# Ghostish/ObjectCentricOccCompletion

Measured on AMD Instinct MI355X. Metric: object-grids/sec (fwd+bwd), higher is better.
Workload: dtype bf16; 1 GPU; configs[1]: SubMConv3d-only occupancy encoder fwd+bwd+AdamW, 64 object grids/GPU x 2000 random points, 0.2 m voxels, 40^3 grid, channels 16-32-64-128, LN+GELU, bf16 features; grids_per_gpu=64, points_per_grid=2000, active_voxels=126005, rulebook_pairs=221211, parallelism=dp1, launch=one hipGraphLaunch per step

## Files before the change

### objectcentricocccompletion_amd/csrc/grid_geometry.hip

```cpp
#include "common.hpp"
#include "row_order.hpp"

namespace {

#ifdef OCOCC_GEO_STAMPS
__device__ long long* g_stamps = nullptr;
#define STAMP(slot) do { if (threadIdx.x == 0 && g_stamps) g_stamps[(int64_t)blockIdx.x * 16 + (slot)] = (long long)__builtin_amdgcn_s_memrealtime(); } while (0)
#else
#define STAMP(slot) do { } while (0)
#endif

constexpr int kThreads = 1024;
constexpr int kWaves = kThreads / 64;
constexpr int kEmitThreads = 256;
constexpr int kEmitWaves = kEmitThreads / 64;
constexpr int kFusedBasesMaxEntries = 256;
#ifndef OCOCC_GEO_FUSED_BASES
#define OCOCC_GEO_FUSED_BASES 1
#endif
constexpr int kPadBlocks = 64;
constexpr int kCols = 28;
constexpr int kMaxSlices = 16;
constexpr int kCodesPerThread = 8;

#define LDS_BARRIER() asm volatile("s_waitcnt lgkmcnt(0)\n\ts_barrier" ::: "memory")

struct GeoParams {
  float vx, vy, vz, xmin, ymin, zmin;
  int32_t gx, gy, gz, batch;
  int32_t words;
  int32_t slices;
  int32_t wps;
  int32_t asplit;
  int32_t spa;
};

__device__ __forceinline__ int32_t lds_rank(const uint32_t* bm, const uint32_t* pf, int32_t cell) {
  const uint32_t w = bm[cell >> 5];
  const uint32_t bit = 1u << (cell & 31);
  return (w & bit) ? (int32_t)(pf[cell >> 5] + __popc(w & (bit - 1u))) : -1;
}

__device__ void lds_popc_scan(const uint32_t* bm, uint32_t* pf, int words, uint32_t* tmp) {
  const int lane = threadIdx.x & 63, wave = threadIdx.x >> 6;
  uint32_t carry = 0;
  for (int w0 = 0; w0 < words; w0 += kThreads) {
    const int w = w0 + threadIdx.x;
    const uint32_t v = w < words ? (uint32_t)__popc(bm[w]) : 0u;
    uint32_t inc = v;
#pragma unroll
    for (int d = 1; d < 64; d <<= 1) {
      const uint32_t t = __shfl_up(inc, d, 64);
      if (lane >= d) inc += t;
    }
    if (lane == 63) tmp[wave] = inc;
    __syncthreads();
    uint32_t before = 0, total = 0;
    for (int t = 0; t < kWaves; ++t) {
      const uint32_t s = tmp[t];
      if (t < wave) before += s;
      total += s;
    }
    if (w < words) pf[w] = carry + before + inc - v;
    carry += total;
    __syncthreads();
  }
}

__device__ void segment_bounds(const int32_t* __restrict__ batch_idx, int64_t n, int32_t key, int64_t* s_two,
                               int64_t* lo_out, int64_t* hi_out) {
  const int64_t step = (n + kThreads - 1) / kThreads;
  if (threadIdx.x < 2) s_two[threadIdx.x] = n;
  __syncthreads();
  {
    const int64_t c0 = (int64_t)threadIdx.x * step;
    if (c0 < n) {
      const int32_t last = batch_idx[(c0 + step < n ? c0 + step : n) - 1];
      const int32_t prev = c0 > 0 ? batch_idx[c0 - 1] : INT32_MIN;
      if (last >= key && prev < key) s_two[0] = c0;
      if (last >= key + 1 && prev < key + 1) s_two[1] = c0;
    }
  }
  __syncthreads();
  const int64_t b0 = s_two[0], b1 = s_two[1];
  __syncthreads();
  if (threadIdx.x < 2) s_two[threadIdx.x] = n;
  __syncthreads();
  for (int64_t t = threadIdx.x; t < 2 * step; t += kThreads) {
    const int which = t >= step;
    const int64_t base = which ? b1 : b0;
    const int64_t i = base + (which ? t - step : t);
    if (base < n && i < n) {
      const int32_t kk = key + which;
      if (batch_idx[i] >= kk && (i == 0 || batch_idx[i - 1] < kk)) s_two[which] = i;
// ... 151 lines not shown
    int32_t v[8], sum = 0;
#pragma unroll
    for (int j = 0; j < 8; ++j) {
      const int64_t e = e0 + (int64_t)lane * 8 + j;
      v[j] = e < entries ? table[e * kCols + c] : 0;
    }
#pragma unroll
    for (int j = 0; j < 8; ++j) sum += v[j];
    int32_t inc = sum;
#pragma unroll
    for (int d = 1; d < 64; d <<= 1) {
      const int32_t t = __shfl_up(inc, d, 64);
      if (lane >= d) inc += t;
    }
    int32_t run = carry + inc - sum;
#pragma unroll
    for (int j = 0; j < 8; ++j) {
      const int64_t e = e0 + (int64_t)lane * 8 + j;
      if (e < entries) bases[e * kCols + c] = run;
      run += v[j];
    }
    carry += __shfl(inc, 63, 64);
  }
  if (lane == 0) {
    totals[c] = carry;
    if (c < 27) indice_num[26 - c] = carry;
    else *num_voxels = (int32_t)(carry < cap ? carry : cap);
  }
}

__device__ __forceinline__ void put_feat_row(const float* __restrict__ src, float* __restrict__ dst_f32,
                                             uint16_t* __restrict__ dst_bf16, int c, float scale) {
  if ((c & 3) == 0) {
    for (int c0 = 0; c0 < c; c0 += 4) {
      float4 v = *(const float4*)(src + c0);
      v.x *= scale; v.y *= scale; v.z *= scale; v.w *= scale;
      *(float4*)(dst_f32 + c0) = v;
      if (dst_bf16) {
        uint2 q;
        q.x = (uint32_t)ococc_f32_to_bf16(v.x) | ((uint32_t)ococc_f32_to_bf16(v.y) << 16);
        q.y = (uint32_t)ococc_f32_to_bf16(v.z) | ((uint32_t)ococc_f32_to_bf16(v.w) << 16);
        *(uint2*)(dst_bf16 + c0) = q;
      }
    }
  } else {
    for (int ch = 0; ch < c; ++ch) {
      const float v = src[ch] * scale;
      dst_f32[ch] = v;
      if (dst_bf16) dst_bf16[ch] = ococc_f32_to_bf16(v);
    }
  }
}

__global__ void __launch_bounds__(kEmitThreads)
grid_emit_kernel(const float* __restrict__ feats, int c, int64_t n, GeoParams g, const uint32_t* __restrict__ bitmap,
                 const uint32_t* __restrict__ local_prefix, uint32_t* __restrict__ prefix_out,
                 int32_t* __restrict__ code_of, const int64_t* __restrict__ seg, const int32_t* __restrict__ bases,
                 const int32_t* __restrict__ totals, int32_t* __restrict__ inv, int32_t* __restrict__ out_coors,
                 int32_t* __restrict__ counts, float* __restrict__ out_f32, uint16_t* __restrict__ out_bf16, int64_t cap,
                 int32_t* __restrict__ nbr_t, uint32_t* __restrict__ blockmask, int32_t* __restrict__ pairs,
                 int emit_blocks, uint32_t* __restrict__ order_hist, i32x4_t* __restrict__ order_rowrec,
                 const int32_t* __restrict__ count_table, const int32_t* __restrict__ part_sums, int32_t* __restrict__ indice_num,
                 int32_t* __restrict__ num_voxels,
                 const int32_t* __restrict__ bad_flags, int nflags, int32_t* __restrict__ status) {
  extern __shared__ uint32_t smem[];
  __shared__ int32_t s_part[3][kEmitWaves][32];
  __shared__ uint32_t s_oh[kLocalBuckets];
  if ((int)blockIdx.x >= emit_blocks) {
    int64_t total;
    if (part_sums) {
      int32_t v = 0;
      for (int e = threadIdx.x; e < g.batch * g.asplit; e += kEmitThreads) v += part_sums[(int64_t)e * kCols + 27];
#pragma unroll
      for (int d = 32; d >= 1; d >>= 1) v += __shfl_xor(v, d, 64);
      if ((threadIdx.x & 63) == 0) s_part[0][threadIdx.x >> 6][0] = v;
      __syncthreads();
      total = 0;
      for (int w = 0; w < kEmitWaves; ++w) total += s_part[0][w][0];
    } else {
      total = totals[27];
    }
    const int64_t turn = (int64_t)(gridDim.x - emit_blocks) * kEmitThreads;
    const int64_t r0 = total + (int64_t)(blockIdx.x - emit_blocks) * kEmitThreads;
    if (r0 >= cap) return;
    for (int64_t r = r0 + threadIdx.x; r - threadIdx.x < cap; r += turn) {
      const bool have = r < cap;
      if (have) {
        *(int4*)(out_coors + r * 4) = make_int4(-1, -1, -1, -1);
        counts[r] = 0;
        for (int ch = 0; ch < c; ++ch) {
          out_f32[r * c + ch] = 0.f;
          if (out_bf16) out_bf16[r * c + ch] = 0;
        }
        for (int k = 0; k < 27; ++k) nbr_t[(int64_t)k * cap + r] = -1;
      }
      if (order_hist) {
        const int key = order_global(order_key_local(0u, 13), (int)blockIdx.x);
        const unsigned long long m = __ballot(have);
        if (m) {
          const int leader = __ffsll((long long)m) - 1;
          uint32_t first = 0u;
          if ((int)(threadIdx.x & 63) == leader) first = atomicAdd(&order_hist[key], (uint32_t)__popcll(m));
          first = __shfl(first, leader, 64);
          const uint32_t place = first + (uint32_t)__builtin_amdgcn_mbcnt_hi((uint32_t)(m >> 32), __builtin_amdgcn_mbcnt_lo((uint32_t)m, 0u));
          if (have) order_rowrec[r] = i32x4_t{(int)((uint32_t)key | (place << kOrderKeyBits)), 0, -1, -1};
        }
      }
    }
    return;
  }
  uint32_t* bm = smem;
  uint32_t* pf = smem + g.words;
  __shared__ int32_t s_base[kCols];
  __shared__ int32_t s_wcnt[27][kEmitWaves];
  __shared__ int32_t s_run[27];
  __shared__ int2 s_list[kCodesPerThread * kEmitThreads];
  __shared__ int s_n, s_n2;
  __shared__ int32_t s_cell[kEmitThreads];
  __shared__ int32_t s_code[kCodesPerThread * kEmitThreads];
  const int b = blockIdx.x / g.slices, sl = blockIdx.x % g.slices;
  const int lane = threadIdx.x & 63, wave = threadIdx.x >> 6;

  STAMP(5);
  constexpr int kPartLoads = kFusedBasesMaxEntries / (2 * kEmitWaves);
  constexpr int kOwnLoads = kMaxSlices / 4;
  int32_t pv[kPartLoads], pw[kOwnLoads];
  const int pcol = threadIdx.x & 31, ppart = threadIdx.x >> 5;
  if (part_sums) {
#pragma unroll
    for (int u = 0; u < kPartLoads; ++u) {
      const int e = ppart + u * 2 * kEmitWaves;
      pv[u] = (pcol < kCols && e < g.batch * g.asplit) ? part_sums[(int64_t)e * kCols + pcol] : 0;
    }
#pragma unroll
    for (int u = 0; u < kOwnLoads; ++u) {
      const int s2 = (sl / g.spa) * g.spa + u;
      pw[u] = (pcol < kCols && ppart == 0 && s2 < sl) ? count_table[((int64_t)b * g.slices + s2) * kCols + pcol] : 0;
    }
  }
  const int64_t p_lo = seg[2 * b], p_hi = seg[2 * b + 1];
  {
    int32_t codes[kCodesPerThread];
#pragma unroll
    for (int j = 0; j < kCodesPerThread; ++j) {
      const int64_t i = p_lo + (int64_t)j * kEmitThreads + threadIdx.x;
      codes[j] = i < p_hi ? code_of[i] : -1;
    }
#pragma unroll
    for (int j = 0; j < kCodesPerThread; ++j) s_code[j * kEmitThreads + threadIdx.x] = codes[j];
  }
  for (int w = threadIdx.x; w < g.words; w += kEmitThreads) {
    bm[w] = bitmap[(int64_t)b * g.words + w];
    pf[w] = local_prefix[(int64_t)b * g.words + w];
  }
  if (part_sums) {
    const int mine = b * g.asplit + sl / g.spa, first = b * g.asplit;
    int32_t a_me = 0, a_grid = 0, a_all = 0;
#pragma unroll
    for (int u = 0; u < kOwnLoads; ++u) a_me += pw[u];
#pragma unroll
    for (int u = 0; u < kPartLoads; ++u) {
      const int e = ppart + u * 2 * kEmitWaves;
      a_me += e < mine ? pv[u] : 0;
      a_grid += e < first ? pv[u] : 0;
      a_all += pv[u];
    }
    a_me += __shfl_xor(a_me, 32, 64);
    a_grid += __shfl_xor(a_grid, 32, 64);
    a_all += __shfl_xor(a_all, 32, 64);
    if (lane < 32) {
      s_part[0][wave][lane] = a_me;
      s_part[1][wave][lane] = a_grid;
      s_part[2][wave][lane] = a_all;
    }
  } else if (threadIdx.x < kCols) {
    s_base[threadIdx.x] = bases[((int64_t)b * g.slices + sl) * kCols + threadIdx.x];
  }
  if (threadIdx.x < 27) s_run[threadIdx.x] = 0;
  if (order_hist)
    for (int i = threadIdx.x; i < kLocalBuckets; i += kEmitThreads) s_oh[i] = 0u;
  int32_t grid_base = part_sums ? 0 : bases[((int64_t)b * g.slices) * kCols + 27];
  __syncthreads();
  if (part_sums) {
#pragma unroll
    for (int w = 0; w < kEmitWaves; ++w) {
      grid_base += s_part[1][w][27];
    }
    if (threadIdx.x < kCols) {
      int32_t me = 0, all = 0;
#pragma unroll
      for (int w = 0; w < kEmitWaves; ++w) {
        me += s_part[0][w][threadIdx.x];
        all += s_part[2][w][threadIdx.x];
      }
      s_base[threadIdx.x] = me;
      if (blockIdx.x == 0) {
        if (threadIdx.x < 27) indice_num[26 - threadIdx.x] = all;
        else *num_voxels = (int32_t)(all < cap ? all : cap);
      }
    }
    if (blockIdx.x == 0 && wave == 1) {
      int bad = 0;
      for (int i = lane; i < nflags; i += 64) bad |= bad_flags[i];
      const unsigned long long m = __ballot(bad != 0);
      if (lane == 0) *status = m ? 1 : 0;
    }
  }
  const int w_lo = sl * g.wps < g.words ? sl * g.wps : g.words, w_hi = (w_lo + g.wps < g.words) ? w_lo + g.wps : g.words;
  const int32_t grid_rows = (int32_t)(pf[g.words - 1] + __popc(bm[g.words - 1]));
  const int32_t row_lo = grid_base + (w_lo < g.words ? (int32_t)pf[w_lo] : grid_rows);
  const int32_t row_hi = grid_base + (w_hi < g.words ? (int32_t)pf[w_hi] : grid_rows);
  for (int w = w_lo + threadIdx.x; w < w_hi; w += kEmitThreads) prefix_out[(int64_t)b * g.words + w] = (uint32_t)grid_base + pf[w];

  STAMP(6);
  const int nrows = row_hi - row_lo;
  const int plane = g.gx * g.gy;
  for (int r0 = 0; r0 < nrows; r0 += kEmitThreads) {
    const int rl = r0 + threadIdx.x;
    const bool have = rl < nrows;
    const int32_t row = row_lo + rl;
    for (int w = w_lo + threadIdx.x; w < w_hi; w += kEmitThreads) {
      uint32_t bits = bm[w];
      int idx = (int)pf[w] - (row_lo - grid_base) - r0;
      if (idx >= kEmitThreads || idx + 32 <= 0) continue;
      while (bits) {
        const int bb = __ffs(bits) - 1;
        bits &= bits - 1;
        if ((unsigned)idx < (unsigned)kEmitThreads) s_cell[idx] = w * 32 + bb;
        ++idx;
      }
    }
    LDS_BARRIER();
    int32_t cell = 0;
    int x = 0, y = 0, z = 0;
    if (have) {
      cell = s_cell[threadIdx.x];
      x = cell % g.gx; y = (cell / g.gx) % g.gy; z = cell / plane;
      if (row < cap) {
        *(int4*)(out_coors + (int64_t)row * 4) = make_int4(b, z, y, x);
        counts[row] = 1;
      }
    }
    int32_t nb[27];
#pragma unroll
    for (int k = 0; k < 27; ++k) nb[k] = -1;
    if (have) {
#pragma unroll
      for (int kz = 0; kz < 3; ++kz)
#pragma unroll
        for (int ky = 0; ky < 3; ++ky) {
          const int zz = z + kz - 1, yy = y + ky - 1;
          if ((unsigned)zz >= (unsigned)g.gz || (unsigned)yy >= (unsigned)g.gy) continue;
          const int32_t c0 = cell + (kz - 1) * plane + (ky - 1) * g.gx - 1;
          const int32_t cs = c0 < 0 ? 0 : c0;
          const int sh = (cs & 31) - (c0 < 0 ? 1 : 0);
          const int wq = cs >> 5;
          const uint32_t wl = bm[wq];
          const uint32_t wh = ((cs & 31) > 29 && wq + 1 < g.words) ? bm[wq + 1] : 0u;
          const unsigned long long both = ((unsigned long long)wh << 32) | wl;
          const uint32_t pre = pf[wq];
#pragma unroll
          for (int kx = 0; kx < 3; ++kx) {
            const int pos = sh + kx;
            if ((unsigned)(x + kx - 1) < (unsigned)g.gx && pos >= 0 && ((both >> pos) & 1ull))
              nb[(kz * 3 + ky) * 3 + kx] = grid_base + (int32_t)(pre + (uint32_t)__popcll(both & ((1ull << pos) - 1ull)));
          }
        }
    }
    STAMP(11);
    uint32_t mbits = 0;
#pragma unroll
    for (int k = 0; k < 27; ++k) {
      if (have && row < cap) nbr_t[(int64_t)k * cap + row] = nb[k];
      const unsigned long long m = __ballot(nb[k] >= 0);
      if (lane == 0) s_wcnt[k][wave] = (int32_t)__popcll(m);
      if (nb[k] >= 0) mbits |= 1u << k;
    }
    if (order_hist && have && row < cap) {
      int32_t e1 = -1, e2 = -1;
#pragma unroll
      for (int k = 0; k < 27; ++k)
        if (k != 13 && nb[k] >= 0) {
          if (e1 < 0) e1 = nb[k];
          else if (e2 < 0) e2 = nb[k];
        }
      const int key = order_key_local(mbits, 13);
      const uint32_t rank = atomicAdd(&s_oh[key], 1u);
      order_rowrec[row] = i32x4_t{(int)((uint32_t)order_global(key, (int)blockIdx.x) | (rank << kOrderKeyBits)),
                                  (int)mbits, e1, e2};
    }
    STAMP(12);
    {
      uint32_t v = mbits;
      const int32_t blk = have ? (row >> 4) : -1 - lane;
#pragma unroll
      for (int d = 1; d < 16; d <<= 1) {
        const uint32_t o = __shfl_down(v, d, 64);
        const int32_t ob = __shfl_down(blk, d, 64);
        if (lane + d < 64 && ob == blk) v |= o;
      }
      const int32_t pb = __shfl_up(blk, 1, 64);
      if (have && row < cap && v && (lane == 0 || pb != blk)) atomicOr(blockmask + blk, v);
    }
    STAMP(13);
    LDS_BARRIER();
    if (threadIdx.x < 27) {
      int32_t acc = s_base[threadIdx.x] + s_run[threadIdx.x];
      const int32_t start = acc;
      for (int t = 0; t < kEmitWaves; ++t) {
        const int32_t cnt = s_wcnt[threadIdx.x][t];
        s_wcnt[threadIdx.x][t] = acc;
        acc += cnt;
      }
      s_run[threadIdx.x] += acc - start;
    }
    LDS_BARRIER();
    STAMP(14);
#pragma unroll
    for (int k = 0; k < 27; ++k) {
      if (nb[k] >= 0) {
        const unsigned long long m = __ballot(true);
        const int32_t p = s_wcnt[k][wave] + (int32_t)__builtin_amdgcn_mbcnt_hi((uint32_t)(m >> 32), __builtin_amdgcn_mbcnt_lo((uint32_t)m, 0u));
        if (p < cap) {
          pairs[((int64_t)(26 - k) * 2 + 0) * cap + p] = row;
          pairs[((int64_t)(26 - k) * 2 + 1) * cap + p] = nb[k];
        }
      }
    }
    LDS_BARRIER();
  }

  constexpr int kOrderPer = (kLocalBuckets + kEmitThreads - 1) / kEmitThreads;
  uint32_t o_cnt[kOrderPer], o_got[kOrderPer];
  if (order_hist) {
    __syncthreads();
#pragma unroll
    for (int i = 0; i < kOrderPer; ++i) {
      const int bk = threadIdx.x + kEmitThreads * i;
      o_cnt[i] = bk < kLocalBuckets ? s_oh[bk] : 0u;
      o_got[i] = 0u;
      if (o_cnt[i]) o_got[i] = atomicAdd(&order_hist[order_global(bk, (int)blockIdx.x)], o_cnt[i]);
    }
  }
  STAMP(7);
  const int32_t cells = g.words * 32;
  const int64_t per_round = (int64_t)kCodesPerThread * kEmitThreads;
  const bool one_round = p_hi - p_lo <= per_round;
  const int pieces = (c + 3) / 4;
  auto load_codes = [&](int64_t base) {
    int32_t codes[kCodesPerThread];
#pragma unroll
    for (int j = 0; j < kCodesPerThread; ++j) {
      const int64_t i = base + (int64_t)j * kEmitThreads + threadIdx.x;
      codes[j] = i < p_hi ? code_of[i] : -1;
    }
#pragma unroll
    for (int j = 0; j < kCodesPerThread; ++j) s_code[j * kEmitThreads + threadIdx.x] = codes[j];
  };
  for (int64_t base = p_lo; base < p_hi; base += per_round) {
    if (base != p_lo) load_codes(base);
    if (threadIdx.x == 0) s_n = 0;
    LDS_BARRIER();
#pragma unroll 1
    for (int j = 0; j < kCodesPerThread; ++j) {
      const int64_t i = base + (int64_t)j * kEmitThreads + threadIdx.x;
      const int32_t code = s_code[j * kEmitThreads + threadIdx.x];
      if (i >= p_hi) continue;
      if (code < 0) {
        if (sl == 0 && code == -2) inv[i] = -1;
        continue;
      }
      const int32_t r = grid_base + lds_rank(bm, pf, (code >> 1) - b * cells);
      if (r < row_lo || r >= row_hi) continue;
      inv[i] = r;
      if (!(code & 1) && r < cap) {
        const int slot = atomicAdd(&s_n, 1);
        s_list[slot] = make_int2((int)(i - p_lo), r);
      }
    }
    LDS_BARRIER();
    const int nl = s_n;
    for (int t = threadIdx.x; t < nl * pieces; t += kEmitThreads) {
      const int2 e = s_list[t / pieces];
      const int piece = t % pieces;
      const float* src = feats + (p_lo + e.x) * c;
      float* dst = out_f32 + (int64_t)e.y * c;
      uint16_t* dst16 = out_bf16 ? out_bf16 + (int64_t)e.y * c : nullptr;
      if ((c & 3) == 0) {
        const float4 v = *(const float4*)(src + piece * 4);
        *(float4*)(dst + piece * 4) = v;
        if (dst16) {
          uint2 q;
          q.x = (uint32_t)ococc_f32_to_bf16(v.x) | ((uint32_t)ococc_f32_to_bf16(v.y) << 16);
          q.y = (uint32_t)ococc_f32_to_bf16(v.z) | ((uint32_t)ococc_f32_to_bf16(v.w) << 16);
          *(uint2*)(dst16 + piece * 4) = q;
        }
      } else {
        for (int ch = piece * 4; ch < piece * 4 + 4 && ch < c; ++ch) {
          dst[ch] = src[ch];
          if (dst16) dst16[ch] = ococc_f32_to_bf16(src[ch]);
        }
      }
    }
    LDS_BARRIER();
  }
  __syncthreads();
  STAMP(8);
  int32_t* s_nfin = &s_n2;
  if (threadIdx.x == 0) s_n2 = 0;
  for (int64_t base = p_lo; base < p_hi; base += per_round) {
    if (!one_round) load_codes(base);
    if (threadIdx.x == 0) s_n = 0;
    LDS_BARRIER();
#pragma unroll 1
    for (int j = 0; j < kCodesPerThread; ++j) {
      const int64_t i = base + (int64_t)j * kEmitThreads + threadIdx.x;
      const int32_t code = s_code[j * kEmitThreads + threadIdx.x];
      if (i >= p_hi || code < 0 || !(code & 1)) continue;
      const int32_t r = grid_base + lds_rank(bm, pf, (code >> 1) - b * cells);
      if (r < row_lo || r >= row_hi || r >= cap) continue;
      const int slot = atomicAdd(&s_n, 1);
      s_list[slot] = make_int2((int)(i - p_lo), r);
    }
    LDS_BARRIER();
    const int nl = s_n;
    for (int t = threadIdx.x; t < nl * c; t += kEmitThreads) {
      const int2 e = s_list[t / c];
      const int ch = t % c;
      atomicAdd(out_f32 + (int64_t)e.y * c + ch, feats[(p_lo + e.x) * c + ch]);
      if (ch == 0 && atomicAdd(counts + e.y, 1) == 1) {
        code_of[p_lo + e.x] = -3 - e.y;
        atomicAdd(s_nfin, 1);
      }
    }
    LDS_BARRIER();
  }
  __syncthreads();
  STAMP(9);
  if (s_n2 > 0) {
    for (int64_t base = p_lo; base < p_hi; base += per_round) {
      load_codes(base);
      if (threadIdx.x == 0) s_n = 0;
      LDS_BARRIER();
#pragma unroll 1
      for (int j = 0; j < kCodesPerThread; ++j) {
        const int64_t i = base + (int64_t)j * kEmitThreads + threadIdx.x;
        const int32_t code = s_code[j * kEmitThreads + threadIdx.x];
        if (i >= p_hi || code > -3) continue;
        const int32_t r = -3 - code;
        if (r < row_lo || r >= row_hi) continue;
        const int slot = atomicAdd(&s_n, 1);
        s_list[slot] = make_int2((int)(i - p_lo), r);
      }
      LDS_BARRIER();
      const int nl = s_n;
      for (int t = threadIdx.x; t < nl * c; t += kEmitThreads) {
        const int64_t r = s_list[t / c].y;
        const int ch = t % c;
        const float cnt = (float)__hip_atomic_load(counts + r, __ATOMIC_RELAXED, __HIP_MEMORY_SCOPE_AGENT);
        const float v = __hip_atomic_load(out_f32 + r * c + ch, __ATOMIC_RELAXED, __HIP_MEMORY_SCOPE_AGENT) / cnt;
        out_f32[r * c + ch] = v;
        if (out_bf16) out_bf16[r * c + ch] = ococc_f32_to_bf16(v);
      }
      LDS_BARRIER();
    }
  }
  STAMP(10);
  if (order_hist) {
#pragma unroll
    for (int i = 0; i < kOrderPer; ++i) {
      const int bk = threadIdx.x + kEmitThreads * i;
      if (o_cnt[i]) s_oh[bk] = o_got[i];
    }
    __syncthreads();
    const int32_t hi = row_hi < cap ? row_hi : (int32_t)cap;
    for (int32_t r = row_lo + threadIdx.x; r < hi; r += kEmitThreads) {
      const uint32_t x = (uint32_t)order_rowrec[r].x;
      const int lk = order_local((int)(x & ((1u << kOrderKeyBits) - 1u)));
      order_rowrec[r].x = (int)(x + (s_oh[lk] << kOrderKeyBits));
    }
  }
}

struct GeoLayout {
  int64_t words_total, off_bitmap, off_prefix, off_code, off_lpre, off_table, off_bases, off_totals, off_seg, off_bad, total;
};

inline bool make_geo_layout(int64_t n, int32_t batch, const int32_t* grid_zyx, int32_t slices, GeoLayout* L,
                            int64_t* grid_unique_total) {
  if (n < 0 || batch < 1 || !grid_zyx || slices < 1 || slices > kMaxSlices) return false;
  int64_t cells = 1;
  for (int i = 0; i < 3; ++i) {
    if (grid_zyx[i] < 1) return false;
    cells *= grid_zyx[i];
  }
  if (cells % 32 != 0 || cells * batch >= (1LL << 30)) return false;
  const int64_t words = cells / 32;
  if (words * 8 > 128 * 1024) return false;
  L->words_total = words * batch;
  const int32_t dims[4] = {batch, grid_zyx[0], grid_zyx[1], grid_zyx[2]};
  const int64_t gu = ococc_grid_unique_workspace_bytes(4, dims);
  if (gu < 0) return false;
  *grid_unique_total = gu;
  L->off_bitmap = 0;
  L->off_prefix = ococc_align_up(L->words_total * 4, 256);
  L->off_code = gu;
  L->off_lpre = L->off_code + ococc_align_up(n * 4, 256);
  L->off_table = L->off_lpre + ococc_align_up(L->words_total * 4, 256);
  const int64_t entries = (int64_t)batch * slices;
  L->off_bases = L->off_table + ococc_align_up(entries * kCols * 4, 256);
  L->off_totals = L->off_bases + ococc_align_up(entries * kCols * 4, 256);
  L->off_seg = L->off_totals + 256;
  L->off_bad = L->off_seg + ococc_align_up((int64_t)batch * 16, 256);
  L->total = L->off_bad + ococc_align_up((int64_t)batch * kMaxSlices * 4, 256);
  return true;
}

}

#ifdef OCOCC_GEO_STAMPS
extern "C" int ococc_geo_set_stamps(long long* dev_buffer) {
  return hipMemcpyToSymbol(HIP_SYMBOL(g_stamps), &dev_buffer, sizeof(dev_buffer)) == hipSuccess ? 0 : -1;
}
#endif

extern "C" int64_t ococc_object_grid_geometry_workspace_bytes(int64_t n, int32_t batch_size,
                                                              const int32_t host_grid_zyx[3], int32_t slices) {
  GeoLayout L;
  int64_t gu;
  if (!make_geo_layout(n, batch_size, host_grid_zyx, slices, &L, &gu)) return -1;
  return L.total;
}

extern "C" int ococc_object_grid_geometry_order_f32(const float* points, int32_t num_point_features, const int32_t* batch_idx,
// ... 2 lines not shown
                                                    const int32_t host_grid_zyx[3], int32_t slices, int32_t* voxel_coors,
                                                    int64_t capacity, int32_t* inv, int32_t* counts, float* voxel_feats,
                                                    uint16_t* voxel_feats_bf16, int32_t* num_voxels, int32_t* status,
                                                    int32_t* nbr_t, uint32_t* blockmask, int32_t* indice_pairs,
                                                    int32_t* indice_num, void* workspace, int64_t workspace_bytes,
                                                    void* order_counters, int32_t* order_rowrec, int32_t* order_rec,
                                                    int32_t* order_hdr, int32_t heavy_blocks, int32_t mid_blocks,
                                                    ococc_stream_t stream_) {
  hipStream_t stream = (hipStream_t)stream_;
  OCOCC_REQUIRE((order_counters == nullptr) == (order_rowrec == nullptr), "order_counters and order_rowrec go together");
  OCOCC_REQUIRE((order_rec == nullptr) == (order_hdr == nullptr) && (!order_rec || order_rowrec),
                "order_rec and order_hdr go together, with order_counters and order_rowrec");
  OCOCC_REQUIRE(!order_rec || ((heavy_blocks == 4 || heavy_blocks == 8 || heavy_blocks == 16) &&
                               (mid_blocks == 4 || mid_blocks == 8 || mid_blocks == 16) && ((uintptr_t)order_rec & 15) == 0),
                "tile sizes must be 4, 8 or 16 blocks; order_rec 16-byte aligned");
  OCOCC_REQUIRE(!order_rowrec || (capacity < kOrderMaxRows && ((uintptr_t)order_rowrec & 15) == 0),
                "row records: 16-byte aligned, below 2^20 rows");
  GeoLayout L;
  int64_t gu;
  OCOCC_REQUIRE(n >= 1 && capacity >= 1 && c >= 1 && num_point_features >= 3, "bad sizes");
  OCOCC_REQUIRE(host_voxel_size && host_coors_range, "null voxel_size / coors_range");
  OCOCC_REQUIRE(make_geo_layout(n, batch_size, host_grid_zyx, slices, &L, &gu),
                "need batch >= 1, grid cells a multiple of 32 and <= 512 Ki per grid, batch * cells < 2^30, 1 <= slices <= 16");
  OCOCC_REQUIRE(num_voxels && status && status == num_voxels + 1, "num_voxels/status: one device int32[2]");
  OCOCC_REQUIRE(points && batch_idx && feats && voxel_coors && inv && counts && voxel_feats && nbr_t && blockmask &&
                    indice_pairs && indice_num, "null device pointer");
  OCOCC_REQUIRE(workspace && workspace_bytes >= L.total, "workspace too small");
  GeoParams g;
  for (int i = 0; i < 3; ++i) {
    OCOCC_REQUIRE(host_voxel_size[i] > 0.f, "voxel size must be positive");
    const int gi = (int)ceilf((host_coors_range[3 + i] - host_coors_range[i]) / host_voxel_size[i]);
    OCOCC_REQUIRE(gi == host_grid_zyx[2 - i], "grid_zyx does not match coors_range / voxel_size");
  }
  g.vx = host_voxel_size[0]; g.vy = host_voxel_size[1]; g.vz = host_voxel_size[2];
  g.xmin = host_coors_range[0]; g.ymin = host_coors_range[1]; g.zmin = host_coors_range[2];
  g.gx = host_grid_zyx[2]; g.gy = host_grid_zyx[1]; g.gz = host_grid_zyx[0];
  g.batch = batch_size;
  g.words = (int32_t)(L.words_total / batch_size);
  g.slices = slices;
  g.wps = (int32_t)ococc_align_up((g.words + slices - 1) / slices, 64);
  g.asplit = slices < 4 ? slices : 4;
  g.spa = (slices + g.asplit - 1) / g.asplit;
  char* ws = (char*)workspace;
  uint32_t* bitmap = (uint32_t*)(ws + L.off_bitmap);
  uint32_t* prefix = (uint32_t*)(ws + L.off_prefix);
  int32_t* code_of = (int32_t*)(ws + L.off_code);
  uint32_t* lpre = (uint32_t*)(ws + L.off_lpre);
  int32_t* table = (int32_t*)(ws + L.off_table);
  int32_t* bases = (int32_t*)(ws + L.off_bases);
  int32_t* totals = (int32_t*)(ws + L.off_totals);
  int64_t* seg = (int64_t*)(ws + L.off_seg);
  int32_t* bad_flags = (int32_t*)(ws + L.off_bad);
  const size_t lds = (size_t)g.words * 8;
  const int64_t mask_words = ococc_cdiv(capacity, 16);
  if (lds > 48 * 1024) {
    OCOCC_HIP(hipFuncSetAttribute((const void*)grid_mark_count_kernel, hipFuncAttributeMaxDynamicSharedMemorySize, (int)lds));
    OCOCC_HIP(hipFuncSetAttribute((const void*)grid_emit_kernel, hipFuncAttributeMaxDynamicSharedMemorySize, (int)lds));
  }
  const bool fused_bases = OCOCC_GEO_FUSED_BASES && (int64_t)batch_size * g.asplit <= kFusedBasesMaxEntries;
  int32_t* part_sums = fused_bases ? bases : nullptr;
  hipLaunchKernelGGL(grid_mark_count_kernel, dim3(batch_size * g.asplit), dim3(kThreads), lds, stream, points,
                     (int)num_point_features, batch_idx, n, g, bitmap, lpre, code_of, table, seg, blockmask, mask_words,
                     inv, bad_flags, (uint32_t*)order_counters, part_sums);
  OCOCC_CHECK_LAUNCH();
  const int64_t entries = (int64_t)batch_size * slices;
  if (!fused_bases) {
    hipLaunchKernelGGL(geometry_bases_kernel, dim3(kCols), dim3(64), 0, stream, table, entries, bases, totals,
                       indice_num, num_voxels, capacity, bad_flags, (int)(batch_size * g.asplit), status);
    OCOCC_CHECK_LAUNCH();
  }
  const int emit_blocks = (int)entries;
  const int64_t pad_need = ococc_cdiv(capacity, kEmitThreads);
  const int pad_blocks = (int)(pad_need < kPadBlocks ? pad_need : kPadBlocks);
  hipLaunchKernelGGL(grid_emit_kernel, dim3(emit_blocks + pad_blocks), dim3(kEmitThreads), lds, stream, feats, (int)c, n, g,
                     bitmap, lpre, prefix, code_of, seg, bases, totals, inv, voxel_coors, counts, voxel_feats,
                     voxel_feats_bf16, capacity, nbr_t, blockmask, indice_pairs, emit_blocks, (uint32_t*)order_counters,
                     (i32x4_t*)order_rowrec, (const int32_t*)table, (const int32_t*)part_sums, indice_num, num_voxels,
                     (const int32_t*)bad_flags, (int)(batch_size * g.asplit), status);
  OCOCC_CHECK_LAUNCH();
  if (order_rec)
    return ococc_subm_row_order_place(order_rowrec, 27, 13, capacity, heavy_blocks, mid_blocks, order_counters, order_rec,
                                      order_hdr, stream_);
  return OCOCC_OK;
}

extern "C" int ococc_object_grid_geometry_f32(const float* points, int32_t num_point_features, const int32_t* batch_idx,
                                              int64_t n, const float* feats, int32_t c, const float host_voxel_size[3],
                                              const float host_coors_range[6], int32_t batch_size,
                                              const int32_t host_grid_zyx[3], int32_t slices, int32_t* voxel_coors,
                                              int64_t capacity, int32_t* inv, int32_t* counts, float* voxel_feats,
                                              uint16_t* voxel_feats_bf16, int32_t* num_voxels, int32_t* status,
                                              int32_t* nbr_t, uint32_t* blockmask, int32_t* indice_pairs,
                                              int32_t* indice_num, void* workspace, int64_t workspace_bytes,
                                              ococc_stream_t stream_) {
  return ococc_object_grid_geometry_order_f32(points, num_point_features, batch_idx, n, feats, c, host_voxel_size,
                                              host_coors_range, batch_size, host_grid_zyx, slices, voxel_coors, capacity, inv,
                                              counts, voxel_feats, voxel_feats_bf16, num_voxels, status, nbr_t, blockmask,
                                              indice_pairs, indice_num, workspace, workspace_bytes, nullptr, nullptr, nullptr,
                                              nullptr, 0, 0, stream_);
}
```

Before: 222,600 object-grids/s.

## Split grid emit into separate row blocks and point-scatter blocks

Moves the per-point work (inv assignment, feature copy, duplicate-voxel atomic averaging) out of the per-slice row-emit blocks into a new set of point blocks, one per grid partition. Each point block loads only its partition of the bitmap and prefix words. Row blocks keep the neighbour, rulebook and order work, and now run without every slice re-scanning all points of the grid. The change also packs the static LDS into explicit structs behind the dynamic bitmap region and adds a waves-per-EU occupancy hint. In exchange it adds more blocks and a larger dynamic LDS request, and it moves counts=1 initialization from the row path to the point path, which could race with the pad initialization.

```diff
diff --git a/objectcentricocccompletion_amd/csrc/grid_geometry.hip b/objectcentricocccompletion_amd/csrc/grid_geometry.hip
--- a/objectcentricocccompletion_amd/csrc/grid_geometry.hip
+++ b/objectcentricocccompletion_amd/csrc/grid_geometry.hip
@@ -22,6 +22,9 @@
 constexpr int kCols = 28;
 constexpr int kMaxSlices = 16;
 constexpr int kCodesPerThread = 8;
+#ifndef OCOCC_GEO_EMIT_WAVES
+#define OCOCC_GEO_EMIT_WAVES 5
+#endif
 
 #define LDS_BARRIER() asm volatile("s_waitcnt lgkmcnt(0)\n\ts_barrier" ::: "memory")
 
@@ -34,12 +37,6 @@
   int32_t asplit;
   int32_t spa;
 };
-
-__device__ __forceinline__ int32_t lds_rank(const uint32_t* bm, const uint32_t* pf, int32_t cell) {
-  const uint32_t w = bm[cell >> 5];
-  const uint32_t bit = 1u << (cell & 31);
-  return (w & bit) ? (int32_t)(pf[cell >> 5] + __popc(w & (bit - 1u))) : -1;
-}
 
 __device__ void lds_popc_scan(const uint32_t* bm, uint32_t* pf, int words, uint32_t* tmp) {
   const int lane = threadIdx.x & 63, wave = threadIdx.x >> 6;
@@ -297,36 +294,52 @@
   }
 }
 
-__global__ void __launch_bounds__(kEmitThreads)
+struct RowLds {
+  int32_t part[3][kEmitWaves][32];
+  uint32_t oh[kLocalBuckets + 3];
+  int32_t base[kCols];
+  int32_t wcnt[27][kEmitWaves];
+  int32_t run[27 + 1];
+  int32_t cell[kEmitThreads];
+};
+struct PointLds {
+  int2 list[kCodesPerThread * kEmitThreads];
+  int32_t code[kCodesPerThread * kEmitThreads];
+  int32_t part[kEmitWaves];
+  int n, n2, pad0, pad1;
+};
+static_assert(sizeof(RowLds) % 16 == 0 && sizeof(PointLds) % 16 == 0, "the bitmap words behind the struct stay aligned");
+
+__global__ void __launch_bounds__(kEmitThreads) __attribute__((amdgpu_waves_per_eu(OCOCC_GEO_EMIT_WAVES)))
 grid_emit_kernel(const float* __restrict__ feats, int c, int64_t n, GeoParams g, const uint32_t* __restrict__ bitmap,
                  const uint32_t* __restrict__ local_prefix, uint32_t* __restrict__ prefix_out,
                  int32_t* __restrict__ code_of, const int64_t* __restrict__ seg, const int32_t* __restrict__ bases,
                  const int32_t* __restrict__ totals, int32_t* __restrict__ inv, int32_t* __restrict__ out_coors,
                  int32_t* __restrict__ counts, float* __restrict__ out_f32, uint16_t* __restrict__ out_bf16, int64_t cap,
                  int32_t* __restrict__ nbr_t, uint32_t* __restrict__ blockmask, int32_t* __restrict__ pairs,
-                 int emit_blocks, uint32_t* __restrict__ order_hist, i32x4_t* __restrict__ order_rowrec,
+                 int emit_blocks, int point_blocks, uint32_t* __restrict__ order_hist, i32x4_t* __restrict__ order_rowrec,
                  const int32_t* __restrict__ count_table, const int32_t* __restrict__ part_sums, int32_t* __restrict__ indice_num,
                  int32_t* __restrict__ num_voxels,
                  const int32_t* __restrict__ bad_flags, int nflags, int32_t* __restrict__ status) {
   extern __shared__ uint32_t smem[];
-  __shared__ int32_t s_part[3][kEmitWaves][32];
-  __shared__ uint32_t s_oh[kLocalBuckets];
-  if ((int)blockIdx.x >= emit_blocks) {
+  RowLds& R = *(RowLds*)smem;
+  if ((int)blockIdx.x >= emit_blocks + point_blocks) {
     int64_t total;
     if (part_sums) {
       int32_t v = 0;
       for (int e = threadIdx.x; e < g.batch * g.asplit; e += kEmitThreads) v += part_sums[(int64_t)e * kCols + 27];
 #pragma unroll
       for (int d = 32; d >= 1; d >>= 1) v += __shfl_xor(v, d, 64);
-      if ((threadIdx.x & 63) == 0) s_part[0][threadIdx.x >> 6][0] = v;
+      if ((threadIdx.x & 63) == 0) R.part[0][threadIdx.x >> 6][0] = v;
       __syncthreads();
       total = 0;
-      for (int w = 0; w < kEmitWaves; ++w) total += s_part[0][w][0];
+      for (int w = 0; w < kEmitWaves; ++w) total += R.part[0][w][0];
     } else {
       total = totals[27];
     }
-    const int64_t turn = (int64_t)(gridDim.x - emit_blocks) * kEmitThreads;
-    const int64_t r0 = total + (int64_t)(blockIdx.x - emit_blocks) * kEmitThreads;
+    const int first_pad = emit_blocks + point_blocks;
+    const int64_t turn = (int64_t)(gridDim.x - first_pad) * kEmitThreads;
+    const int64_t r0 = total + (int64_t)(blockIdx.x - first_pad) * kEmitThreads;
     if (r0 >= cap) return;
     for (int64_t r = r0 + threadIdx.x; r - threadIdx.x < cap; r += turn) {
       const bool have = r < cap;
@@ -354,15 +367,187 @@
     }
     return;
   }
-  uint32_t* bm = smem;
-  uint32_t* pf = smem + g.words;
-  __shared__ int32_t s_base[kCols];
-  __shared__ int32_t s_wcnt[27][kEmitWaves];
-  __shared__ int32_t s_run[27];
-  __shared__ int2 s_list[kCodesPerThread * kEmitThreads];
-  __shared__ int s_n, s_n2;
-  __shared__ int32_t s_cell[kEmitThreads];
-  __shared__ int32_t s_code[kCodesPerThread * kEmitThreads];
+  if ((int)blockIdx.x >= emit_blocks) {
+    PointLds& P = *(PointLds*)smem;
+    uint32_t* bm = smem + sizeof(PointLds) / 4;
+    uint32_t* pf = bm + g.spa * g.wps;
+    const int pblk = (int)blockIdx.x - emit_blocks;
+    const int b = pblk / g.asplit, part = pblk % g.asplit;
+    const int lane = threadIdx.x & 63, wave = threadIdx.x >> 6;
+    STAMP(5);
+    const int64_t p_lo = seg[2 * b], p_hi = seg[2 * b + 1];
+    {
+      int32_t codes[kCodesPerThread];
+#pragma unroll
+      for (int j = 0; j < kCodesPerThread; ++j) {
+        const int64_t i = p_lo + (int64_t)j * kEmitThreads + threadIdx.x;
+        codes[j] = i < p_hi ? code_of[i] : -1;
+      }
+#pragma unroll
+      for (int j = 0; j < kCodesPerThread; ++j) P.code[j * kEmitThreads + threadIdx.x] = codes[j];
+    }
+    const int pw_lo = part * g.spa * g.wps < g.words ? part * g.spa * g.wps : g.words;
+    const int pw_hi = pw_lo + g.spa * g.wps < g.words ? pw_lo + g.spa * g.wps : g.words;
+    const uint32_t* gbm = bitmap + (int64_t)b * g.words;
+    const uint32_t* gpf = local_prefix + (int64_t)b * g.words;
+    for (int w = pw_lo + threadIdx.x; w < pw_hi; w += kEmitThreads) {
+      bm[w - pw_lo] = gbm[w];
+      pf[w - pw_lo] = gpf[w];
+    }
+    int32_t grid_base = 0;
+    if (part_sums) {
+      int32_t v = 0;
+      for (int e = threadIdx.x; e < b * g.asplit; e += kEmitThreads) v += part_sums[(int64_t)e * kCols + 27];
+#pragma unroll
+      for (int d = 32; d >= 1; d >>= 1) v += __shfl_xor(v, d, 64);
+      if (lane == 0) P.part[wave] = v;
+    } else {
+      grid_base = bases[((int64_t)b * g.slices) * kCols + 27];
+    }
+    if (threadIdx.x == 0) P.n2 = 0;
+    const int32_t grid_rows = (int32_t)(gpf[g.words - 1] + __popc(gbm[g.words - 1]));
+    const int32_t loc_lo = pw_lo < g.words ? (int32_t)gpf[pw_lo] : grid_rows;
+    const int32_t loc_hi = pw_hi < g.words ? (int32_t)gpf[pw_hi] : grid_rows;
+    __syncthreads();
+    if (part_sums) {
+#pragma unroll
+      for (int w = 0; w < kEmitWaves; ++w) grid_base += P.part[w];
+    }
+    const int32_t row_lo = grid_base + loc_lo, row_hi = grid_base + loc_hi;
+    auto part_rank = [&](int32_t cell) -> int32_t {
+      const int wi = (cell >> 5) - pw_lo;
+      if ((unsigned)wi >= (unsigned)(pw_hi - pw_lo)) return -1;
+      const uint32_t w = bm[wi];
+      const uint32_t bit = 1u << (cell & 31);
+      return (w & bit) ? grid_base + (int32_t)(pf[wi] + __popc(w & (bit - 1u))) : -1;
+    };
+    STAMP(6);
+    const int32_t cells = g.words * 32;
+    const int64_t per_round = (int64_t)kCodesPerThread * kEmitThreads;
+    const bool one_round = p_hi - p_lo <= per_round;
+    const int pieces = (c + 3) / 4;
+    auto load_codes = [&](int64_t base) {
+      int32_t codes[kCodesPerThread];
+#pragma unroll
+      for (int j = 0; j < kCodesPerThread; ++j) {
+        const int64_t i = base + (int64_t)j * kEmitThreads + threadIdx.x;
+        codes[j] = i < p_hi ? code_of[i] : -1;
+      }
+#pragma unroll
+      for (int j = 0; j < kCodesPerThread; ++j) P.code[j * kEmitThreads + threadIdx.x] = codes[j];
+    };
+    for (int64_t base = p_lo; base < p_hi; base += per_round) {
+      if (base != p_lo) load_codes(base);
+      if (threadIdx.x == 0) P.n = 0;
+      LDS_BARRIER();
+#pragma unroll 1
+      for (int j = 0; j < kCodesPerThread; ++j) {
+        const int64_t i = base + (int64_t)j * kEmitThreads + threadIdx.x;
+        const int32_t code = P.code[j * kEmitThreads + threadIdx.x];
+        if (i >= p_hi) continue;
+        if (code < 0) {
+          if (part == 0 && code == -2) inv[i] = -1;
+          continue;
+        }
+        const int32_t r = part_rank((code >> 1) - b * cells);
+        if (r < 0) continue;
+        inv[i] = r;
+        if (!(code & 1) && r < cap) {
+          const int slot = atomicAdd(&P.n, 1);
+          P.list[slot] = make_int2((int)(i - p_lo), r);
+        }
+      }
+      LDS_BARRIER();
+      const int nl = P.n;
+      for (int t = threadIdx.x; t < nl * pieces; t += kEmitThreads) {
+        const int2 e = P.list[t / pieces];
+        const int piece = t % pieces;
+        const float* src = feats + (p_lo + e.x) * c;
+        float* dst = out_f32 + (int64_t)e.y * c;
+        uint16_t* dst16 = out_bf16 ? out_bf16 + (int64_t)e.y * c : nullptr;
+        if (piece == 0) counts[e.y] = 1;
+        if ((c & 3) == 0) {
+          const float4 v = *(const float4*)(src + piece * 4);
+          *(float4*)(dst + piece * 4) = v;
+          if (dst16) {
+            uint2 q;
+            q.x = (uint32_t)ococc_f32_to_bf16(v.x) | ((uint32_t)ococc_f32_to_bf16(v.y) << 16);
+            q.y = (uint32_t)ococc_f32_to_bf16(v.z) | ((uint32_t)ococc_f32_to_bf16(v.w) << 16);
+            *(uint2*)(dst16 + piece * 4) = q;
+          }
+        } else {
+          for (int ch = piece * 4; ch < piece * 4 + 4 && ch < c; ++ch) {
+            dst[ch] = src[ch];
+            if (dst16) dst16[ch] = ococc_f32_to_bf16(src[ch]);
+          }
+        }
+      }
+      LDS_BARRIER();
+    }
+    __syncthreads();
+    STAMP(8);
+    for (int64_t base = p_lo; base < p_hi; base += per_round) {
+      if (!one_round) load_codes(base);
+      if (threadIdx.x == 0) P.n = 0;
+      LDS_BARRIER();
+#pragma unroll 1
+      for (int j = 0; j < kCodesPerThread; ++j) {
+        const int64_t i = base + (int64_t)j * kEmitThreads + threadIdx.x;
+        const int32_t code = P.code[j * kEmitThreads + threadIdx.x];
+        if (i >= p_hi || code < 0 || !(code & 1)) continue;
+        const int32_t r = part_rank((code >> 1) - b * cells);
+        if (r < 0 || r >= cap) continue;
+        const int slot = atomicAdd(&P.n, 1);
+        P.list[slot] = make_int2((int)(i - p_lo), r);
+      }
+      LDS_BARRIER();
+      const int nl = P.n;
+      for (int t = threadIdx.x; t < nl * c; t += kEmitThreads) {
+        const int2 e = P.list[t / c];
+        const int ch = t % c;
+        atomicAdd(out_f32 + (int64_t)e.y * c + ch, feats[(p_lo + e.x) * c + ch]);
+        if (ch == 0 && atomicAdd(counts + e.y, 1) == 1) {
+          code_of[p_lo + e.x] = -3 - e.y;
+          atomicAdd(&P.n2, 1);
+        }
+      }
+      LDS_BARRIER();
+    }
+    __syncthreads();
+    STAMP(9);
+    if (P.n2 > 0) {
+      for (int64_t base = p_lo; base < p_hi; base += per_round) {
+        load_codes(base);
+        if (threadIdx.x == 0) P.n = 0;
+        LDS_BARRIER();
+#pragma unroll 1
+        for (int j = 0; j < kCodesPerThread; ++j) {
+          const int64_t i = base + (int64_t)j * kEmitThreads + threadIdx.x;
+          const int32_t code = P.code[j * kEmitThreads + threadIdx.x];
+          if (i >= p_hi || code > -3) continue;
+          const int32_t r = -3 - code;
+          if (r < row_lo || r >= row_hi) continue;
+          const int slot = atomicAdd(&P.n, 1);
+          P.list[slot] = make_int2((int)(i - p_lo), r);
+        }
+        LDS_BARRIER();
+        const int nl = P.n;
+        for (int t = threadIdx.x; t < nl * c; t += kEmitThreads) {
+          const int64_t r = P.list[t / c].y;
+          const int ch = t % c;
+          const float cnt = (float)__hip_atomic_load(counts + r, __ATOMIC_RELAXED, __HIP_MEMORY_SCOPE_AGENT);
+          const float v = __hip_atomic_load(out_f32 + r * c + ch, __ATOMIC_RELAXED, __HIP_MEMORY_SCOPE_AGENT) / cnt;
+          out_f32[r * c + ch] = v;
+          if (out_bf16) out_bf16[r * c + ch] = ococc_f32_to_bf16(v);
+        }
+        LDS_BARRIER();
+      }
+    }
+    STAMP(10);
+    return;
+  }
+  uint32_t* bm = smem + sizeof(RowLds) / 4;
+  uint32_t* pf = bm + g.words;
   const int b = blockIdx.x / g.slices, sl = blockIdx.x % g.slices;
   const int lane = threadIdx.x & 63, wave = threadIdx.x >> 6;
 
@@ -383,17 +568,6 @@
       pw[u] = (pcol < kCols && ppart == 0 && s2 < sl) ? count_table[((int64_t)b * g.slices + s2) * kCols + pcol] : 0;
     }
   }
-  const int64_t p_lo = seg[2 * b], p_hi = seg[2 * b + 1];
-  {
-    int32_t codes[kCodesPerThread];
-#pragma unroll
-    for (int j = 0; j < kCodesPerThread; ++j) {
-      const int64_t i = p_lo + (int64_t)j * kEmitThreads + threadIdx.x;
-      codes[j] = i < p_hi ? code_of[i] : -1;
-    }
-#pragma unroll
-    for (int j = 0; j < kCodesPerThread; ++j) s_code[j * kEmitThreads + threadIdx.x] = codes[j];
-  }
   for (int w = threadIdx.x; w < g.words; w += kEmitThreads) {
     bm[w] = bitmap[(int64_t)b * g.words + w];
     pf[w] = local_prefix[(int64_t)b * g.words + w];
@@ -414,31 +588,31 @@
     a_grid += __shfl_xor(a_grid, 32, 64);
     a_all += __shfl_xor(a_all, 32, 64);
     if (lane < 32) {
-      s_part[0][wave][lane] = a_me;
-      s_part[1][wave][lane] = a_grid;
-      s_part[2][wave][lane] = a_all;
+      R.part[0][wave][lane] = a_me;
+      R.part[1][wave][lane] = a_grid;
+      R.part[2][wave][lane] = a_all;
     }
   } else if (threadIdx.x < kCols) {
-    s_base[threadIdx.x] = bases[((int64_t)b * g.slices + sl) * kCols + threadIdx.x];
-  }
-  if (threadIdx.x < 27) s_run[threadIdx.x] = 0;
+    R.base[threadIdx.x] = bases[((int64_t)b * g.slices + sl) * kCols + threadIdx.x];
+  }
+  if (threadIdx.x < 27) R.run[threadIdx.x] = 0;
   if (order_hist)
-    for (int i = threadIdx.x; i < kLocalBuckets; i += kEmitThreads) s_oh[i] = 0u;
+    for (int i = threadIdx.x; i < kLocalBuckets; i += kEmitThreads) R.oh[i] = 0u;
   int32_t grid_base = part_sums ? 0 : bases[((int64_t)b * g.slices) * kCols + 27];
   __syncthreads();
   if (part_sums) {
 #pragma unroll
     for (int w = 0; w < kEmitWaves; ++w) {
-      grid_base += s_part[1][w][27];
+      grid_base += R.part[1][w][27];
     }
     if (threadIdx.x < kCols) {
       int32_t me = 0, all = 0;
 #pragma unroll
       for (int w = 0; w < kEmitWaves; ++w) {
-        me += s_part[0][w][threadIdx.x];
-        all += s_part[2][w][threadIdx.x];
-      }
-      s_base[threadIdx.x] = me;
+        me += R.part[0][w][threadIdx.x];
+        all += R.part[2][w][threadIdx.x];
+      }
+      R.base[threadIdx.x] = me;
       if (blockIdx.x == 0) {
         if (threadIdx.x < 27) indice_num[26 - threadIdx.x] = all;
         else *num_voxels = (int32_t)(all < cap ? all : cap);
@@ -471,7 +645,7 @@
       while (bits) {
         const int bb = __ffs(bits) - 1;
         bits &= bits - 1;
-        if ((unsigned)idx < (unsigned)kEmitThreads) s_cell[idx] = w * 32 + bb;
+        if ((unsigned)idx < (unsigned)kEmitThreads) R.cell[idx] = w * 32 + bb;
         ++idx;
       }
     }
@@ -479,12 +653,9 @@
     int32_t cell = 0;
     int x = 0, y = 0, z = 0;
     if (have) {
-      cell = s_cell[threadIdx.x];
+      cell = R.cell[threadIdx.x];
       x = cell % g.gx; y = (cell / g.gx) % g.gy; z = cell / plane;
-      if (row < cap) {
-        *(int4*)(out_coors + (int64_t)row * 4) = make_int4(b, z, y, x);
-        counts[row] = 1;
-      }
+      if (row < cap) *(int4*)(out_coors + (int64_t)row * 4) = make_int4(b, z, y, x);
     }
     int32_t nb[27];
 #pragma unroll
@@ -518,7 +689,7 @@
     for (int k = 0; k < 27; ++k) {
       if (have && row < cap) nbr_t[(int64_t)k * cap + row] = nb[k];
       const unsigned long long m = __ballot(nb[k] >= 0);
-      if (lane == 0) s_wcnt[k][wave] = (int32_t)__popcll(m);
+      if (lane == 0) R.wcnt[k][wave] = (int32_t)__popcll(m);
       if (nb[k] >= 0) mbits |= 1u << k;
     }
     if (order_hist && have && row < cap) {
@@ -530,7 +701,7 @@
           else if (e2 < 0) e2 = nb[k];
         }
       const int key = order_key_local(mbits, 13);
-      const uint32_t rank = atomicAdd(&s_oh[key], 1u);
+      const uint32_t rank = atomicAdd(&R.oh[key], 1u);
       order_rowrec[row] = i32x4_t{(int)((uint32_t)order_global(key, (int)blockIdx.x) | (rank << kOrderKeyBits)),
                                   (int)mbits, e1, e2};
     }
@@ -550,14 +721,14 @@
     STAMP(13);
     LDS_BARRIER();
     if (threadIdx.x < 27) {
-      int32_t acc = s_base[threadIdx.x] + s_run[threadIdx.x];
+      int32_t acc = R.base[threadIdx.x] + R.run[threadIdx.x];
       const int32_t start = acc;
       for (int t = 0; t < kEmitWaves; ++t) {
-        const int32_t cnt = s_wcnt[threadIdx.x][t];
-        s_wcnt[threadIdx.x][t] = acc;
+        const int32_t cnt = R.wcnt[threadIdx.x][t];
+        R.wcnt[threadIdx.x][t] = acc;
         acc += cnt;
       }
-      s_run[threadIdx.x] += acc - start;
+      R.run[threadIdx.x] += acc - start;
     }
     LDS_BARRIER();
     STAMP(14);
@@ -565,7 +736,7 @@
     for (int k = 0; k < 27; ++k) {
       if (nb[k] >= 0) {
         const unsigned long long m = __ballot(true);
-        const int32_t p = s_wcnt[k][wave] + (int32_t)__builtin_amdgcn_mbcnt_hi((uint32_t)(m >> 32), __builtin_amdgcn_mbcnt_lo((uint32_t)m, 0u));
+        const int32_t p = R.wcnt[k][wave] + (int32_t)__builtin_amdgcn_mbcnt_hi((uint32_t)(m >> 32), __builtin_amdgcn_mbcnt_lo((uint32_t)m, 0u));
         if (p < cap) {
           pairs[((int64_t)(26 - k) * 2 + 0) * cap + p] = row;
           pairs[((int64_t)(26 - k) * 2 + 1) * cap + p] = nb[k];
@@ -582,149 +753,27 @@
 #pragma unroll
     for (int i = 0; i < kOrderPer; ++i) {
       const int bk = threadIdx.x + kEmitThreads * i;
-      o_cnt[i] = bk < kLocalBuckets ? s_oh[bk] : 0u;
+      o_cnt[i] = bk < kLocalBuckets ? R.oh[bk] : 0u;
       o_got[i] = 0u;
       if (o_cnt[i]) o_got[i] = atomicAdd(&order_hist[order_global(bk, (int)blockIdx.x)], o_cnt[i]);
     }
   }
   STAMP(7);
-  const int32_t cells = g.words * 32;
-  const int64_t per_round = (int64_t)kCodesPerThread * kEmitThreads;
-  const bool one_round = p_hi - p_lo <= per_round;
-  const int pieces = (c + 3) / 4;
-  auto load_codes = [&](int64_t base) {
-    int32_t codes[kCodesPerThread];
-#pragma unroll
-    for (int j = 0; j < kCodesPerThread; ++j) {
-      const int64_t i = base + (int64_t)j * kEmitThreads + threadIdx.x;
-      codes[j] = i < p_hi ? code_of[i] : -1;
-    }
-#pragma unroll
-    for (int j = 0; j < kCodesPerThread; ++j) s_code[j * kEmitThreads + threadIdx.x] = codes[j];
-  };
-  for (int64_t base = p_lo; base < p_hi; base += per_round) {
-    if (base != p_lo) load_codes(base);
-    if (threadIdx.x == 0) s_n = 0;
-    LDS_BARRIER();
-#pragma unroll 1
-    for (int j = 0; j < kCodesPerThread; ++j) {
-      const int64_t i = base + (int64_t)j * kEmitThreads + threadIdx.x;
-      const int32_t code = s_code[j * kEmitThreads + threadIdx.x];
-      if (i >= p_hi) continue;
-      if (code < 0) {
-        if (sl == 0 && code == -2) inv[i] = -1;
-        continue;
-      }
-      const int32_t r = grid_base + lds_rank(bm, pf, (code >> 1) - b * cells);
-      if (r < row_lo || r >= row_hi) continue;
-      inv[i] = r;
-      if (!(code & 1) && r < cap) {
-        const int slot = atomicAdd(&s_n, 1);
-        s_list[slot] = make_int2((int)(i - p_lo), r);
-      }
-    }
-    LDS_BARRIER();
-    const int nl = s_n;
-    for (int t = threadIdx.x; t < nl * pieces; t += kEmitThreads) {
-      const int2 e = s_list[t / pieces];
-      const int piece = t % pieces;
-      const float* src = feats + (p_lo + e.x) * c;
-      float* dst = out_f32 + (int64_t)e.y * c;
-      uint16_t* dst16 = out_bf16 ? out_bf16 + (int64_t)e.y * c : nullptr;
-      if ((c & 3) == 0) {
-        const float4 v = *(const float4*)(src + piece * 4);
-        *(float4*)(dst + piece * 4) = v;
-        if (dst16) {
-          uint2 q;
-          q.x = (uint32_t)ococc_f32_to_bf16(v.x) | ((uint32_t)ococc_f32_to_bf16(v.y) << 16);
-          q.y = (uint32_t)ococc_f32_to_bf16(v.z) | ((uint32_t)ococc_f32_to_bf16(v.w) << 16);
-          *(uint2*)(dst16 + piece * 4) = q;
-        }
-      } else {
-        for (int ch = piece * 4; ch < piece * 4 + 4 && ch < c; ++ch) {
-          dst[ch] = src[ch];
-          if (dst16) dst16[ch] = ococc_f32_to_bf16(src[ch]);
-        }
-      }
-    }
-    LDS_BARRIER();
-  }
-  __syncthreads();
-  STAMP(8);
-  int32_t* s_nfin = &s_n2;
-  if (threadIdx.x == 0) s_n2 = 0;
-  for (int64_t base = p_lo; base < p_hi; base += per_round) {
-    if (!one_round) load_codes(base);
-    if (threadIdx.x == 0) s_n = 0;
-    LDS_BARRIER();
-#pragma unroll 1
-    for (int j = 0; j < kCodesPerThread; ++j) {
-      const int64_t i = base + (int64_t)j * kEmitThreads + threadIdx.x;
-      const int32_t code = s_code[j * kEmitThreads + threadIdx.x];
-      if (i >= p_hi || code < 0 || !(code & 1)) continue;
-      const int32_t r = grid_base + lds_rank(bm, pf, (code >> 1) - b * cells);
-      if (r < row_lo || r >= row_hi || r >= cap) continue;
-      const int slot = atomicAdd(&s_n, 1);
-      s_list[slot] = make_int2((int)(i - p_lo), r);
-    }
-    LDS_BARRIER();
-    const int nl = s_n;
-    for (int t = threadIdx.x; t < nl * c; t += kEmitThreads) {
-      const int2 e = s_list[t / c];
-      const int ch = t % c;
-      atomicAdd(out_f32 + (int64_t)e.y * c + ch, feats[(p_lo + e.x) * c + ch]);
-      if (ch == 0 && atomicAdd(counts + e.y, 1) == 1) {
-        code_of[p_lo + e.x] = -3 - e.y;
-        atomicAdd(s_nfin, 1);
-      }
-    }
-    LDS_BARRIER();
-  }
-  __syncthreads();
-  STAMP(9);
-  if (s_n2 > 0) {
-    for (int64_t base = p_lo; base < p_hi; base += per_round) {
-      load_codes(base);
-      if (threadIdx.x == 0) s_n = 0;
-      LDS_BARRIER();
-#pragma unroll 1
-      for (int j = 0; j < kCodesPerThread; ++j) {
-        const int64_t i = base + (int64_t)j * kEmitThreads + threadIdx.x;
-        const int32_t code = s_code[j * kEmitThreads + threadIdx.x];
-        if (i >= p_hi || code > -3) continue;
-        const int32_t r = -3 - code;
-        if (r < row_lo || r >= row_hi) continue;
-        const int slot = atomicAdd(&s_n, 1);
-        s_list[slot] = make_int2((int)(i - p_lo), r);
-      }
-      LDS_BARRIER();
-      const int nl = s_n;
-      for (int t = threadIdx.x; t < nl * c; t += kEmitThreads) {
-        const int64_t r = s_list[t / c].y;
-        const int ch = t % c;
-        const float cnt = (float)__hip_atomic_load(counts + r, __ATOMIC_RELAXED, __HIP_MEMORY_SCOPE_AGENT);
-        const float v = __hip_atomic_load(out_f32 + r * c + ch, __ATOMIC_RELAXED, __HIP_MEMORY_SCOPE_AGENT) / cnt;
-        out_f32[r * c + ch] = v;
-        if (out_bf16) out_bf16[r * c + ch] = ococc_f32_to_bf16(v);
-      }
-      LDS_BARRIER();
-    }
-  }
-  STAMP(10);
   if (order_hist) {
 #pragma unroll
     for (int i = 0; i < kOrderPer; ++i) {
       const int bk = threadIdx.x + kEmitThreads * i;
-      if (o_cnt[i]) s_oh[bk] = o_got[i];
+      if (o_cnt[i]) R.oh[bk] = o_got[i];
     }
     __syncthreads();
     const int32_t hi = row_hi < cap ? row_hi : (int32_t)cap;
     for (int32_t r = row_lo + threadIdx.x; r < hi; r += kEmitThreads) {
       const uint32_t x = (uint32_t)order_rowrec[r].x;
       const int lk = order_local((int)(x & ((1u << kOrderKeyBits) - 1u)));
-      order_rowrec[r].x = (int)(x + (s_oh[lk] << kOrderKeyBits));
-    }
-  }
+      order_rowrec[r].x = (int)(x + (R.oh[lk] << kOrderKeyBits));
+    }
+  }
+  STAMP(15);
 }
 
 struct GeoLayout {
@@ -833,11 +882,13 @@
   int64_t* seg = (int64_t*)(ws + L.off_seg);
   int32_t* bad_flags = (int32_t*)(ws + L.off_bad);
   const size_t lds = (size_t)g.words * 8;
+  const size_t lds_row = sizeof(RowLds) + (size_t)g.words * 8, lds_point = sizeof(PointLds) + (size_t)g.spa * g.wps * 8;
+  const size_t lds_emit = lds_row > lds_point ? lds_row : lds_point;
   const int64_t mask_words = ococc_cdiv(capacity, 16);
-  if (lds > 48 * 1024) {
+  if (lds > 48 * 1024)
     OCOCC_HIP(hipFuncSetAttribute((const void*)grid_mark_count_kernel, hipFuncAttributeMaxDynamicSharedMemorySize, (int)lds));
-    OCOCC_HIP(hipFuncSetAttribute((const void*)grid_emit_kernel, hipFuncAttributeMaxDynamicSharedMemorySize, (int)lds));
-  }
+  if (lds_emit > 48 * 1024)
+    OCOCC_HIP(hipFuncSetAttribute((const void*)grid_emit_kernel, hipFuncAttributeMaxDynamicSharedMemorySize, (int)lds_emit));
   const bool fused_bases = OCOCC_GEO_FUSED_BASES && (int64_t)batch_size * g.asplit <= kFusedBasesMaxEntries;
   int32_t* part_sums = fused_bases ? bases : nullptr;
   hipLaunchKernelGGL(grid_mark_count_kernel, dim3(batch_size * g.asplit), dim3(kThreads), lds, stream, points,
@@ -850,14 +901,14 @@
                        indice_num, num_voxels, capacity, bad_flags, (int)(batch_size * g.asplit), status);
     OCOCC_CHECK_LAUNCH();
   }
-  const int emit_blocks = (int)entries;
+  const int emit_blocks = (int)entries, point_blocks = batch_size * g.asplit;
   const int64_t pad_need = ococc_cdiv(capacity, kEmitThreads);
   const int pad_blocks = (int)(pad_need < kPadBlocks ? pad_need : kPadBlocks);
-  hipLaunchKernelGGL(grid_emit_kernel, dim3(emit_blocks + pad_blocks), dim3(kEmitThreads), lds, stream, feats, (int)c, n, g,
-                     bitmap, lpre, prefix, code_of, seg, bases, totals, inv, voxel_coors, counts, voxel_feats,
-                     voxel_feats_bf16, capacity, nbr_t, blockmask, indice_pairs, emit_blocks, (uint32_t*)order_counters,
-                     (i32x4_t*)order_rowrec, (const int32_t*)table, (const int32_t*)part_sums, indice_num, num_voxels,
-                     (const int32_t*)bad_flags, (int)(batch_size * g.asplit), status);
+  hipLaunchKernelGGL(grid_emit_kernel, dim3(emit_blocks + point_blocks + pad_blocks), dim3(kEmitThreads), lds_emit, stream, feats,
+                     (int)c, n, g, bitmap, lpre, prefix, code_of, seg, bases, totals, inv, voxel_coors, counts, voxel_feats,
+                     voxel_feats_bf16, capacity, nbr_t, blockmask, indice_pairs, emit_blocks, point_blocks,
+                     (uint32_t*)order_counters, (i32x4_t*)order_rowrec, (const int32_t*)table, (const int32_t*)part_sums,
+                     indice_num, num_voxels, (const int32_t*)bad_flags, (int)(batch_size * g.asplit), status);
   OCOCC_CHECK_LAUNCH();
   if (order_rec)
     return ococc_subm_row_order_place(order_rowrec, 27, 13, capacity, heavy_blocks, mid_blocks, order_counters, order_rec,
```

Result: faster. 228,300 object-grids/s (median of 6 runs) (+2.6%).
